# xyfJASON/ctrlora

Measured on NVIDIA H100. Metric: ddim_steps_per_sec, higher is better.
Workload: dtype fp16 (fp32 accumulate)

## Files before the change

ctrlora_b200/csrc/attention_sm90.cu:

```cuda
#include "common.cuh"
#include "ctrlora_b200.h"
#include "wgmma.cuh"
#include <math.h>
#include <string.h>

namespace ctrl {

int make_tmap_f16(CUtensorMap* map, const void* base, int rank, const uint64_t* dims, const uint64_t* strides_bytes,
                  const uint32_t* box);
int persistent_sms();

struct AttnParams {
    int Nq, Nk, heads, d;
    int n_kv_tiles, q_tiles, units;
    float scale_log2e;
    __half* out;
    long long ldo;
    float* lse;
};

constexpr int ATT_BKV = 64;

template <int DP>
struct AttnSmem {
    static constexpr int NWG = DP <= 48 ? 3 : 2;
    static constexpr int BQ = 64 * NWG;
    static constexpr int THREADS = 128 * (NWG + 1), CONSUMERS = 128 * NWG;
    static constexpr int PRODUCER_REGS = NWG == 3 ? 24 : 40, CONSUMER_REGS = NWG == 3 ? 160 : 232;
    static constexpr int NKC = (DP + 63) / 64;
    static constexpr int STAGES = DP <= 48 ? 6 : DP <= 80 ? 4 : 3;
    static constexpr int Q_CHUNK = BQ * 128;
    static constexpr int Q_BYTES = NKC * Q_CHUNK;
    static constexpr int K_CHUNK = ATT_BKV * 128;
    static constexpr int K_BYTES = NKC * K_CHUNK;
    static constexpr int V_BYTES = DP * 128;
    static constexpr int STAGE = K_BYTES + V_BYTES;
    static constexpr int DATA = Q_BYTES + STAGES * STAGE;
    static constexpr int TOTAL = DATA + (2 + 2 * STAGES) * 8 + 1024;
};

template <int DP>
__device__ __forceinline__ void issue_qk(float* s, uint32_t sQ, uint32_t sK) {
    using L = AttnSmem<DP>;
#pragma unroll
    for (int kk = 0; kk < DP / 16; ++kk)
        WgmmaSS<64, 0, 0>::mma(s, wgmma_desc_kmajor(sQ + (kk >> 2) * L::Q_CHUNK + (kk & 3) * 32),
                               wgmma_desc_kmajor(sK + (kk >> 2) * L::K_CHUNK + (kk & 3) * 32), kk ? 1u : 0u);
    wgmma_commit();
}

template <int DP>
__device__ __forceinline__ void issue_pv(float* o, const uint32_t* pa, uint32_t sV) {
#pragma unroll
    for (int kk = 0; kk < 4; ++kk) WgmmaRS<DP, 0>::mma(o, pa + 4 * kk, wgmma_desc_kmajor(sV + 32 * kk), 1u);
    wgmma_commit();
}

template <bool MASK>
__device__ __forceinline__ void softmax_tile(float* s, float (&m)[2], float (&l)[2], float (&a)[2], float c, int key0,
                                             int nk) {
    float mx[2] = {m[0], m[1]};
#pragma unroll
    for (int i = 0; i < 8; ++i)
#pragma unroll
        for (int e = 0; e < 2; ++e) {
            const bool ok = !MASK || key0 + 8 * i + e < nk;
            s[4 * i + e] = ok ? s[4 * i + e] * c : -INFINITY;
            s[4 * i + 2 + e] = ok ? s[4 * i + 2 + e] * c : -INFINITY;
            mx[0] = fmaxf(mx[0], s[4 * i + e]);
            mx[1] = fmaxf(mx[1], s[4 * i + 2 + e]);
        }
    float ls[2] = {0.f, 0.f};
#pragma unroll
    for (int h = 0; h < 2; ++h) {
        mx[h] = fmaxf(mx[h], __shfl_xor_sync(0xffffffffu, mx[h], 1));
        mx[h] = fmaxf(mx[h], __shfl_xor_sync(0xffffffffu, mx[h], 2));
        a[h] = fast_exp2(m[h] - mx[h]);
        m[h] = mx[h];
    }
#pragma unroll
    for (int i = 0; i < 8; ++i)
#pragma unroll
        for (int e = 0; e < 2; ++e) {
            s[4 * i + e] = fast_exp2(s[4 * i + e] - m[0]);
            s[4 * i + 2 + e] = fast_exp2(s[4 * i + 2 + e] - m[1]);
            ls[0] += s[4 * i + e];
            ls[1] += s[4 * i + 2 + e];
        }
    l[0] = l[0] * a[0] + ls[0];
    l[1] = l[1] * a[1] + ls[1];
}

__device__ __forceinline__ void pack_a_frags(const float* x, uint32_t* a) {
#pragma unroll
    for (int i = 0; i < 8; ++i) {
        a[4 * (i >> 1) + 2 * (i & 1)] = pack_half2(x[4 * i], x[4 * i + 1]);
        a[4 * (i >> 1) + 2 * (i & 1) + 1] = pack_half2(x[4 * i + 2], x[4 * i + 3]);
    }
}

template <int DP>
__global__ void __launch_bounds__(AttnSmem<DP>::THREADS, 1)
attention_kernel(const __grid_constant__ CUtensorMap tmQ, const __grid_constant__ CUtensorMap tmK,
                 const __grid_constant__ CUtensorMap tmV, const __grid_constant__ AttnParams p) {
    using L = AttnSmem<DP>;
    extern __shared__ uint8_t smem_raw[];
    uint8_t* smem = reinterpret_cast<uint8_t*>((reinterpret_cast<uintptr_t>(smem_raw) + 1023) & ~uintptr_t(1023));
    uint64_t* q_full = reinterpret_cast<uint64_t*>(smem + L::DATA);
    uint64_t* q_empty = q_full + 1;
    uint64_t* full = q_full + 2;
    uint64_t* empty = full + L::STAGES;
    pdl_launch_dependents();
    const int warp = uniform_warp_idx();
    const int n_kv = p.n_kv_tiles;
    if (threadIdx.x == 0) {
        tma_prefetch_desc(&tmQ);
        tma_prefetch_desc(&tmK);
        tma_prefetch_desc(&tmV);
        mbar_init(q_full, 1);
        mbar_init(q_empty, L::CONSUMERS);
        for (int i = 0; i < L::STAGES; ++i) {
            mbar_init(&full[i], 1);
            mbar_init(&empty[i], L::CONSUMERS);
        }
        fence_barrier_init();
    }
    __syncthreads();
    pdl_wait();

    if (warp < 4) {
        setmaxnreg_dec<L::PRODUCER_REGS>();
        if (warp == 0 && elect_one()) {
            int s = 0;
            uint32_t phase = 0, qphase = 0;
            for (int u = blockIdx.x; u < p.units; u += gridDim.x) {
                const int qt = u % p.q_tiles, hi = u / p.q_tiles, head = hi % p.heads, img = hi / p.heads;
                mbar_wait_nocall(q_empty, qphase ^ 1);
                qphase ^= 1;
                mbar_expect_tx(q_full, L::Q_BYTES);
#pragma unroll
                for (int c = 0; c < L::NKC; ++c)
                    tma_load_4d(smem + c * L::Q_CHUNK, &tmQ, q_full, c * 64, head, qt * L::BQ, img);
                for (int t = 0; t < n_kv; ++t) {
                    mbar_wait_nocall(&empty[s], phase ^ 1);
                    uint8_t* dst = smem + L::Q_BYTES + s * L::STAGE;
                    mbar_expect_tx(&full[s], L::STAGE);
#pragma unroll
                    for (int c = 0; c < L::NKC; ++c)
                        tma_load_4d(dst + c * L::K_CHUNK, &tmK, &full[s], c * 64, head, t * ATT_BKV, img);
                    tma_load_4d(dst + L::K_BYTES, &tmV, &full[s], t * ATT_BKV, 0, head, img);
                    if (++s == L::STAGES) { s = 0; phase ^= 1; }
                }
            }
        }
        return;
    }

    setmaxnreg_inc<L::CONSUMER_REGS>();
    const int ct = threadIdx.x - 128, wg = ct >> 7, lane = threadIdx.x & 31;
    const uint32_t sQ = smem_u32(smem) + wg * 64 * 128, sKV = smem_u32(smem) + L::Q_BYTES;
    const float c = p.scale_log2e;
    const bool ragged = (p.Nk % ATT_BKV) != 0;
    const int kq = 2 * (lane & 3);
    const int bar_own = 1 + wg, bar_next = 1 + (wg + 1) % L::NWG;
    if (wg == L::NWG - 1) named_bar_arrive(1, 256);
    int s = 0;
    uint32_t phase = 0, qphase = 0;
    for (int u = blockIdx.x; u < p.units; u += gridDim.x) {
        const int qt = u % p.q_tiles, hi = u / p.q_tiles, head = hi % p.heads, img = hi / p.heads;
        float o[DP / 2];
#pragma unroll
        for (int i = 0; i < DP / 2; ++i) o[i] = 0.f;
        float m[2] = {-INFINITY, -INFINITY}, l[2] = {0.f, 0.f}, a[2];
        float sc[32];
        uint32_t pa[16];
        mbar_wait_nocall(q_full, qphase);
        qphase ^= 1;

        mbar_wait_nocall(&full[s], phase);
        named_bar_sync(bar_own, 256);
        wgmma_fence();
        issue_qk<DP>(sc, sQ, sKV + s * L::STAGE);
        named_bar_arrive(bar_next, 256);
        wgmma_wait<0>();
        wgmma_fence_regs<32>(sc);
        if (n_kv == 1) mbar_arrive(q_empty);
        if (ragged && n_kv == 1) softmax_tile<true>(sc, m, l, a, c, kq, p.Nk);
        else softmax_tile<false>(sc, m, l, a, c, kq, p.Nk);
        pack_a_frags(sc, pa);
        int prev = s;
        if (++s == L::STAGES) { s = 0; phase ^= 1; }

        for (int t = 1; t < n_kv; ++t) {
            mbar_wait_nocall(&full[s], phase);
            named_bar_sync(bar_own, 256);
            wgmma_fence();
            issue_qk<DP>(sc, sQ, sKV + s * L::STAGE);
            issue_pv<DP>(o, pa, sKV + prev * L::STAGE + L::K_BYTES);
            named_bar_arrive(bar_next, 256);
            wgmma_wait<1>();
            wgmma_fence_regs<32>(sc);
            if (t == n_kv - 1) mbar_arrive(q_empty);
            if (ragged && t == n_kv - 1) softmax_tile<true>(sc, m, l, a, c, t * ATT_BKV + kq, p.Nk);
            else softmax_tile<false>(sc, m, l, a, c, t * ATT_BKV + kq, p.Nk);
            wgmma_wait<0>();
            wgmma_fence_regs<DP / 2>(o);
            wgmma_fence_regs<16>(pa);
            mbar_arrive(&empty[prev]);
            if (__any_sync(0xffffffffu, a[0] != 1.f || a[1] != 1.f)) {
#pragma unroll
                for (int i = 0; i < DP / 8; ++i) {
                    o[4 * i] *= a[0]; o[4 * i + 1] *= a[0];
                    o[4 * i + 2] *= a[1]; o[4 * i + 3] *= a[1];
                }
            }
            pack_a_frags(sc, pa);
            prev = s;
            if (++s == L::STAGES) { s = 0; phase ^= 1; }
        }
        wgmma_fence();
        issue_pv<DP>(o, pa, sKV + prev * L::STAGE + L::K_BYTES);
        wgmma_wait<0>();
        wgmma_fence_regs<DP / 2>(o);
        mbar_arrive(&empty[prev]);

#pragma unroll
        for (int h = 0; h < 2; ++h) {
            l[h] += __shfl_xor_sync(0xffffffffu, l[h], 1);
            l[h] += __shfl_xor_sync(0xffffffffu, l[h], 2);
        }
        const float inv0 = 1.0f / l[0], inv1 = 1.0f / l[1];
        const int r0 = qt * L::BQ + wg * 64 + ((ct >> 5) & 3) * 16 + (lane >> 2), r1 = r0 + 8;
        __half* o0 = p.out + (static_cast<long long>(img) * p.Nq + r0) * p.ldo + head * p.d;
        __half* o1 = p.out + (static_cast<long long>(img) * p.Nq + r1) * p.ldo + head * p.d;
#pragma unroll
        for (int i = 0; i < DP / 8; ++i) {
            const int col = 8 * i + kq;
            if (col >= p.d) continue;
            if (r0 < p.Nq) *reinterpret_cast<__half2*>(o0 + col) = __floats2half2_rn(o[4 * i] * inv0, o[4 * i + 1] * inv0);
            if (r1 < p.Nq) *reinterpret_cast<__half2*>(o1 + col) = __floats2half2_rn(o[4 * i + 2] * inv1, o[4 * i + 3] * inv1);
        }
        if (p.lse && (lane & 3) == 0) {
            float* lrow = p.lse + (static_cast<long long>(img) * p.heads + head) * p.Nq;
            if (r0 < p.Nq) lrow[r0] = m[0] + log2f(l[0]);
            if (r1 < p.Nq) lrow[r1] = m[1] + log2f(l[1]);
        }
    }
    if (wg == 0) named_bar_sync(1, 256);
}

template <int DP>
static int launch_attn(const CUtensorMap& tq, const CUtensorMap& tk, const CUtensorMap& tv, const AttnParams& p, int grid,
                       cudaStream_t stream) {
    using L = AttnSmem<DP>;
    static bool attr = false;
    if (!attr) {
        if (cudaFuncSetAttribute(attention_kernel<DP>, cudaFuncAttributeMaxDynamicSharedMemorySize, L::TOTAL) != cudaSuccess)
            return CTRLORA_ERR_CUDA;
        attr = true;
    }
    if (launch_pdl(attention_kernel<DP>, dim3(grid), dim3(L::THREADS), (size_t)L::TOTAL, stream, tq, tk, tv, p) !=
        cudaSuccess)
        return CTRLORA_ERR_CUDA;
    return cudaGetLastError() == cudaSuccess ? CTRLORA_OK : CTRLORA_ERR_CUDA;
}

}

using namespace ctrl;

extern "C" int ctrlora_attention_f16(const void* q, long long ldq, const void* k, long long ldk, const void* vt,
                                     int nk_pad, void* out, long long ldo, float* lse, int batch, int heads, int nq,
                                     int nk, int head_dim, void* stream_) {
    cudaStream_t stream = reinterpret_cast<cudaStream_t>(stream_);
    if (!q || !k || !vt || !out) return CTRLORA_ERR_ARG;
    const int d = head_dim;
    if (d % 8 != 0 || d > 160 || nk_pad % 8 != 0 || nk_pad < nk || ldq % 8 != 0 || ldk % 8 != 0 || ldo % 8 != 0 || nk < 1)
        return CTRLORA_ERR_ARG;
    const int dp = d <= 48 ? 48 : d <= 80 ? 80 : 160;
    const int bq = dp == 48 ? AttnSmem<48>::BQ : dp == 80 ? AttnSmem<80>::BQ : AttnSmem<160>::BQ;
    AttnParams p;
    memset(&p, 0, sizeof(p));
    p.Nq = nq; p.Nk = nk; p.heads = heads; p.d = d;
    p.n_kv_tiles = (nk + ATT_BKV - 1) / ATT_BKV;
    p.q_tiles = (nq + bq - 1) / bq;
    p.units = p.q_tiles * heads * batch;
    p.scale_log2e = (1.0f / sqrtf(static_cast<float>(d))) * 1.4426950408889634f;
    p.out = reinterpret_cast<__half*>(out); p.ldo = ldo; p.lse = lse;
    if (p.units == 0) return CTRLORA_OK;
    const int sms = persistent_sms();
    if (sms <= 0) return CTRLORA_ERR_CUDA;
    CUtensorMap tq, tk, tv;
    {
        uint64_t dims[4] = {(uint64_t)d, (uint64_t)heads, (uint64_t)nq, (uint64_t)batch};
        uint64_t str[3] = {(uint64_t)d * 2, (uint64_t)ldq * 2, (uint64_t)ldq * 2 * nq};
        uint32_t box[4] = {64, 1, (uint32_t)bq, 1};
        int rc = make_tmap_f16(&tq, q, 4, dims, str, box);
        if (rc) return rc;
    }
    {
        uint64_t dims[4] = {(uint64_t)d, (uint64_t)heads, (uint64_t)nk, (uint64_t)batch};
        uint64_t str[3] = {(uint64_t)d * 2, (uint64_t)ldk * 2, (uint64_t)ldk * 2 * nk};
        uint32_t box[4] = {64, 1, ATT_BKV, 1};
        int rc = make_tmap_f16(&tk, k, 4, dims, str, box);
        if (rc) return rc;
    }
    {
        uint64_t dims[4] = {(uint64_t)nk, (uint64_t)d, (uint64_t)heads, (uint64_t)batch};
        uint64_t str[3] = {(uint64_t)nk_pad * 2, (uint64_t)nk_pad * 2 * d, (uint64_t)nk_pad * 2 * d * heads};
        uint32_t box[4] = {ATT_BKV, (uint32_t)dp, 1, 1};
        int rc = make_tmap_f16(&tv, vt, 4, dims, str, box);
        if (rc) return rc;
    }
    const int grid = p.units < sms ? p.units : sms;
    if (dp == 48) return launch_attn<48>(tq, tk, tv, p, grid, stream);
    if (dp == 80) return launch_attn<80>(tq, tk, tv, p, grid, stream);
    return launch_attn<160>(tq, tk, tv, p, grid, stream);
}
```

ctrlora_b200/ops.py:

```python
import ctypes as C

import torch

from . import _lib
from ._lib import GemmArgs, check


LAUNCHES = 0
_GEMM_PROFILE = None
_GEMM_SHAPES = None
_GEMM_RECORD = None


def _count(n=1):
    global LAUNCHES
    LAUNCHES += n


def _ungraphed(fn, sampler):
    old = getattr(sampler, "use_cuda_graph", False)
    if sampler is not None:
        sampler.use_cuda_graph = False
    try:
        fn()
# ... 157 lines not shown
        assert residual.dtype in (torch.float16, torch.float32) and residual.stride(-1) == 1
        args.residual, args.ldr = _ptr(residual), residual.stride(-2)
        args.residual_f32 = int(residual.dtype == torch.float32)
    args.out_scale, args.head_dim, args.tok_pad, args.bf16 = float(out_scale), head_dim, tok_pad, 0
    ws, cnt = _splitk_buffers(a.device)
    args.split_k, args.splitk_ws, args.splitk_ws_bytes = split_k, ws.data_ptr(), SPLITK_WS_BYTES
    args.splitk_counters, args.splitk_counters_len = cnt.data_ptr(), SPLITK_COUNTERS
    if dup_out is not None:
        args.dup_out, args.dup_ld = dup_out.data_ptr(), dup_out.stride(0)
    args.force_single_cta = int(single_cta)
    args.relu = int(bool(relu))
    if hi is not None:
        if hi.get("rowbias") is not None:
            assert rowbias is not None and hi["rowbias"].stride(0) == rowbias.stride(0) and \
                hi["rowbias"].stride(-1) == 1, "the two halves' row terms need one row stride"
        args.group_b, args.w_hi, args.w2_hi = b // 2, _ptr(hi["w"]), _ptr(hi.get("w2"))
        args.bias_hi, args.rowbias_hi = _ptr(hi.get("bias")), _ptr(hi.get("rowbias"))
    lib = _lib.load()
    shape = {"B": b, "H": h, "W": wd, "C": c, "N": n_rows, "ksize": ksize, "geglu": int(geglu),
             "c2": int(args.a2_c) if a2 is not None else 0, "segs": seg_width, "res": int(residual is not None)}
    keep = (a, w, a2, w2, bias, rowbias, residual, out, seg_outs, dup_out, ws, cnt, hi)
    if _launch_gemm(lib.ctrlora_gemm_f16_simt if simt else lib.ctrlora_gemm_f16, args, simt, shape, keep):
        return ret
    half = a.shape[0] // 2
    rows = half if a.dim() == 2 else half * a.shape[1] * a.shape[2]
    imgs = rows // (rows_per_img or rows)

    def cut(t, lo, by_image=False):
        if t is None:
            return None
        n = imgs if by_image else (half if t.dim() == 4 else rows)
        return t[:n] if lo else t[n:]

    for lo in (True, False):
        segs = None if seg_outs is None else [cut(o, lo, by_image=bool(t)) for o, t in zip(seg_outs, transposed)]
        _gemm(cut(a, lo), w if lo else hi["w"], ksize=ksize, bias=bias if lo else hi.get("bias"),
              rowbias=rowbias if lo else hi.get("rowbias"), rows_per_img=rows_per_img, rowbias_ld=rowbias_ld,
              residual=cut(residual, lo), out_scale=out_scale, a2=cut(a2, lo), w2=w2 if lo else hi.get("w2"),
              geglu=geglu, out=cut(out, lo), out_f32=out_f32, seg_outs=segs, seg_width=seg_width, transposed=transposed,
              head_dim=head_dim, tok_pad=tok_pad, block_n=block_n, split_k=split_k, relu=relu)
    return ret


def _launch_gemm(fn, args, simt, shape, keep):
    flops = 2.0 * shape["B"] * shape["H"] * shape["W"] * shape["N"] * (shape["ksize"] ** 2 * shape["C"] + shape["c2"])
    timed = _GEMM_PROFILE is not None and not simt
    if timed:
        e0, e1 = torch.cuda.Event(enable_timing=True), torch.cuda.Event(enable_timing=True)
        e0.record()
    rc = fn(C.addressof(args), _sp())
    if rc == _lib.STATUS_UNSUPPORTED and args.group_b:
        return False
    check(rc, "ctrlora_gemm_f16")
    _count()
    if _GEMM_RECORD is not None and not simt:
        _GEMM_RECORD.append((args, flops, keep))
    if timed:
        e1.record()
        _GEMM_PROFILE.append((flops, e0, e1))
        if _GEMM_SHAPES is not None:
            _GEMM_SHAPES.append(shape)
    return True


def _dp(t):
    return t.data_ptr() if t is not None else None


def _sp():
    return torch.cuda.current_stream().cuda_stream


_GN_PARTIAL = {}
GN_PARTIAL_FLOATS = 1 << 19
GN_PARTIAL_COUNTERS = 256


def _gn_partial_buffers(device):
    key = device.index if device.index is not None else torch.cuda.current_device()
    if key not in _GN_PARTIAL:
        if torch.cuda.is_current_stream_capturing():
            raise _lib.CtrloraError("the GroupNorm partial-statistics scratch is allocated on the first call on a device; "
                                    "make one un-captured GroupNorm call before capturing a graph")
        _GN_PARTIAL[key] = (torch.empty(GN_PARTIAL_FLOATS, device=device, dtype=torch.float32),
                            torch.zeros(GN_PARTIAL_COUNTERS, device=device, dtype=torch.int32))
    return _GN_PARTIAL[key]


def _gn_args(x1, gamma, beta, eps, silu, add1, add1_scale, x2, add2, add2_scale, groups):
    b, h, w, c1, ld1 = _as_bhwc(x1)
    c2, ld2 = 0, 0
    if x2 is not None:
        b2, h2, w2, c2, ld2 = _as_bhwc(x2)
        assert (b2, h2, w2) == (b, h, w)
    a = _lib.GroupNormArgs()
    a.x1, a.add1, a.add1_scale, a.c1, a.ld1 = _dp(x1), _dp(add1), float(add1_scale), c1, ld1
    a.x2, a.add2, a.add2_scale, a.c2, a.ld2 = _dp(x2), _dp(add2), float(add2_scale), c2, ld2
    a.batch, a.hw, a.groups = b, h * w, groups
    a.gamma, a.beta, a.eps, a.silu = _dp(gamma), _dp(beta), float(eps), int(silu)
    pws, pcnt = _gn_partial_buffers(x1.device)
    a.partial_ws, a.partial_ws_floats = _dp(pws), GN_PARTIAL_FLOATS
    a.partial_counters, a.partial_counters_len = _dp(pcnt), GN_PARTIAL_COUNTERS
    return a, (b, h, w, c1, c2)


def groupnorm(x1, gamma, beta, eps, silu, *, add1=None, add1_scale=1.0, x2=None, add2=None, add2_scale=1.0,
              groups=32, want_raw=False, want_stats=False, out=None, gamma_hi=None, beta_hi=None):
    _require_cuda(x1, x2, add1, add2)
    a, (b, h, w, c1, c2) = _gn_args(x1, gamma, beta, eps, silu, add1, add1_scale, x2, add2, add2_scale, groups)
    for ad, ref in ((add1, x1), (add2, x2)):
        if ad is not None:
            assert ad.shape == ref.shape and ad.stride() == ref.stride() and ad.dtype == torch.float16
    ctot = c1 + c2
    y = torch.empty((b, h, w, ctot), device=x1.device, dtype=torch.float16) if out is None else out
    assert y.shape == (b, h, w, ctot) and y.is_contiguous() and y.dtype == torch.float16
    raw = torch.empty_like(y) if want_raw else None
    stats_ws = torch.empty(b * groups * 2, device=x1.device, dtype=torch.float32)
    a.stats_ws = _dp(stats_ws)
    assert gamma.dtype == torch.float32 and beta.dtype == torch.float32 and gamma.numel() == ctot
    if gamma_hi is not None:
        assert b % 2 == 0 and gamma_hi.numel() == ctot and beta_hi.numel() == ctot
        a.gamma_hi, a.beta_hi, a.group_b = _dp(gamma_hi), _dp(beta_hi), b // 2
    a.y, a.raw_out = _dp(y), _dp(raw)
    _count(2)
    check(_lib.load().ctrlora_groupnorm_f16(C.addressof(a), _sp()), "ctrlora_groupnorm_f16")
    if want_stats:
        return (y, raw, stats_ws) if want_raw else (y, stats_ws)
    return (y, raw) if want_raw else y


def zeros(shape, device, dtype=torch.float16):
    t = torch.empty(shape, device=device, dtype=dtype)
    check(_lib.load().ctrlora_memset_zero(_dp(t), t.numel() * t.element_size(), _sp()), "memset_zero")
    return t


def layernorm(x, gamma, beta, eps=1e-5, gamma_hi=None, beta_hi=None):
    _require_cuda(x)
    cols = x.shape[-1]
    x2 = x.reshape(-1, cols)
    y = torch.empty((x2.shape[0], cols), device=x.device, dtype=torch.float16)
    _count(1)
    if gamma_hi is not None:
        assert x2.shape[0] % 2 == 0
        check(_lib.load().ctrlora_layernorm_grouped_f16(_dp(x2), x2.stride(0), _dp(y), cols, x2.shape[0], cols, _dp(gamma),
                                                        _dp(beta), _dp(gamma_hi), _dp(beta_hi), x2.shape[0] // 2,
                                                        float(eps), _sp()), "ctrlora_layernorm_grouped_f16")
        return y.view(x.shape)
    check(_lib.load().ctrlora_layernorm_f16(_dp(x2), x2.stride(0), _dp(y), cols, x2.shape[0], cols, _dp(gamma), _dp(beta),
                                            float(eps), _sp()), "ctrlora_layernorm_f16")
    return y.view(x.shape)


def attention(q, k, vt, batch, heads, nq, nk, head_dim, out=None, lse=None):
    _require_cuda(q, k, vt)
    if out is None:
        out = torch.empty((batch * nq, heads * head_dim), device=q.device, dtype=torch.float16)
    _count(1)
    check(_lib.load().ctrlora_attention_f16(_dp(q), q.stride(0), _dp(k), k.stride(0), _dp(vt), vt.shape[-1], _dp(out),
                                            out.stride(0), _dp(lse), batch, heads, nq, nk, head_dim, _sp()),
          "ctrlora_attention_f16")
    return out


def nchw_to_nhwc_f16(x, c_pad=None, out=None):
    _require_cuda(x)
    assert x.dtype == torch.float32 and x.is_contiguous()
    b, c, h, w = x.shape
    c_pad = c_pad or c
    y = torch.empty((b, h, w, c_pad), device=x.device, dtype=torch.float16) if out is None else out
    assert y.shape == (b, h, w, c_pad) and y.is_contiguous() and y.dtype == torch.float16
    _count(1)
    check(_lib.load().ctrlora_nchw_f32_to_nhwc_f16(_dp(x), _dp(y), b, c, h * w, c_pad, _sp()), "nchw_to_nhwc")
    return y


def nhwc_to_nchw_f32(x, channels=None):
    _require_cuda(x)
    b, h, w, c, ld = _as_bhwc(x)
    channels = channels or c
    y = torch.empty((b, channels, h, w), device=x.device, dtype=torch.float32)
    _count(1)
    check(_lib.load().ctrlora_nhwc_to_nchw_f32(_dp(x), int(x.dtype == torch.float32), ld, _dp(y), b, channels, h * w,
                                               _sp()), "nhwc_to_nchw")
    return y


def timestep_embedding(t, freqs):
    _require_cuda(t, freqs)
    assert t.dtype in (torch.int64, torch.float32) and freqs.dtype == torch.float32
    out = torch.empty((t.shape[0], 2 * freqs.shape[0]), device=t.device, dtype=torch.float32)
    fn = _lib.load().ctrlora_timestep_embedding if t.dtype == torch.int64 else _lib.load().ctrlora_timestep_embedding_f32
    _count(1)
    check(fn(_dp(t), _dp(freqs), _dp(out), t.shape[0], freqs.shape[0], _sp()), "timestep_embedding")
    return out


def small_linear(x, w, bias, silu_in=False, silu_out=False, out=None):
    _require_cuda(x, w)
    assert x.dtype == torch.float32 and w.dtype == torch.float16 and w.is_contiguous() and x.stride(1) == 1
    rows, k = x.shape
    n = w.shape[0]
    if out is None:
        out = torch.empty((rows, n), device=x.device, dtype=torch.float32)
    _count(1)
    check(_lib.load().ctrlora_small_linear(_dp(x), x.stride(0), _dp(w), _dp(bias), _dp(out), out.stride(0), rows, n, k,
                                           int(silu_in), int(silu_out), _sp()), "small_linear")
    return out


def upsample2x(x):
    _require_cuda(x)
    assert x.is_contiguous() and x.dtype == torch.float16
    b, h, w, c = x.shape
    y = torch.empty((b, 2 * h, 2 * w, c), device=x.device, dtype=torch.float16)
    _count(1)
    check(_lib.load().ctrlora_upsample2x_f16(_dp(x), _dp(y), b, h, w, c, _sp()), "upsample2x")
    return y


def im2col_s2(x, pad_lo=1):
    _require_cuda(x)
    assert x.is_contiguous() and x.dtype == torch.float16
    b, h, w, c = x.shape
    y = torch.empty((b, h // 2, w // 2, 9 * c), device=x.device, dtype=torch.float16)
    _count(1)
    check(_lib.load().ctrlora_im2col_s2_pad_f16(_dp(x), _dp(y), b, h, w, c, int(pad_lo), _sp()), "im2col_s2")
    return y


def softmax_rows(logits, scale=1.0):
    _require_cuda(logits)
    assert logits.dtype == torch.float32 and logits.dim() == 2 and logits.stride(1) == 1
    out = torch.empty(logits.shape, device=logits.device, dtype=torch.float16)
    _count(1)
    check(_lib.load().ctrlora_softmax_rows_f32_to_f16(_dp(logits), logits.stride(0), _dp(out), out.stride(0), logits.shape[0],
                                                      logits.shape[1], float(scale), _sp()), "softmax_rows")
    return out


def gaussian_sample(moments, noise=None, scale=1.0):
    _require_cuda(moments, noise)
    moments = moments.float().contiguous()
    b, z2, h, w = moments.shape
    out = torch.empty((b, z2 // 2, h, w), device=moments.device, dtype=torch.float32)
    if noise is not None:
        noise = noise.float().contiguous()
        assert noise.shape == out.shape
    _count(1)
    check(_lib.load().ctrlora_gaussian_sample(_dp(moments), _dp(noise), _dp(out), b, z2 // 2, h * w, float(scale), _sp()),
          "gaussian_sample")
    return out


def cast_transpose(src, batch, rows, cols, out=None):
    _require_cuda(src)
    assert src.dtype == torch.float32 and src.is_contiguous() and src.numel() == batch * rows * cols
    if out is None:
        out = torch.empty((batch, cols, rows), device=src.device, dtype=torch.float16)
    _count(1)
    check(_lib.load().ctrlora_cast_transpose_f32_to_f16(_dp(src), _dp(out), batch, rows, cols, _sp()), "cast_transpose")
    return out


def ddim_update(x, e_cond, e_uncond, cfg_scale, a_t, a_prev, sigma_t, sqrt_one_minus_at, noise=None, temperature=1.0,
                stats=None):
    _require_cuda(x, e_cond, e_uncond, noise)
    for t in (x, e_cond, e_uncond, noise):
        assert t is None or (t.dtype == torch.float32 and t.is_contiguous() and t.shape == x.shape)
    x_prev, pred_x0 = torch.empty_like(x), torch.empty_like(x)
    b = x.shape[0]
    _count(1)
    check(_lib.load().ctrlora_ddim_update(_dp(x), _dp(e_cond), _dp(e_uncond), _dp(noise), _dp(x_prev), _dp(pred_x0),
                                          _dp(stats), b, x[0].numel(), float(cfg_scale), float(a_t), float(a_prev),
                                          float(sigma_t), float(sqrt_one_minus_at), float(temperature), _sp()),
          "ddim_update")
    return x_prev, pred_x0


def im2col_3x3(x):
    _require_cuda(x)
    assert x.is_contiguous() and x.dtype == torch.float16
    b, h, w, c = x.shape
    y = torch.empty((b, h, w, 9 * c), device=x.device, dtype=torch.float16)
    _count()
    check(_lib.load().ctrlora_im2col_3x3_f16(_dp(x), _dp(y), b, h, w, c, _sp()), "im2col_3x3")
    return y


def outer_accum(dy, x, out, alpha=1.0, beta=1.0, silu_x=False):
    _require_cuda(dy, x, out)
    assert dy.dtype == x.dtype == out.dtype == torch.float32 and dy.stride(1) == 1 and x.stride(1) == 1 and out.stride(1) == 1
    rows, n = dy.shape
    k = x.shape[1]
    assert x.shape[0] == rows and out.shape == (n, k)
    _count()
    check(_lib.load().ctrlora_outer_accum_f32(_dp(dy), dy.stride(0), _dp(x), x.stride(0), _dp(out), out.stride(0), rows, n, k,
                                              float(alpha), float(beta), int(silu_x), _sp()), "outer_accum")
    return out


def copy2d(src, dst, rows, cols, lds, ldd, accumulate=False):
    _require_cuda(src, dst)
    assert src.dtype == dst.dtype == torch.float32
    _count()
    check(_lib.load().ctrlora_copy2d_f32(_dp(src), lds, _dp(dst), ldd, rows, cols, int(accumulate), _sp()), "copy2d")
    return dst


def silu_bwd(d, x):
# ... 704 lines not shown
```

ctrlora_b200/train.py:

```python
import numbers
import os

import torch
import torch.nn as nn

from . import checkpoint, ops, prepare
from .runtime import nchw_view, pixel_major, to_f16_rows

f32 = prepare.bias_f32


class GradSink:

    def __init__(self, control_model, named=None):
        if named is None:
            from cldm.cldm_ctrlora_finetune import trainable_parameters
            if not getattr(control_model, "ft_with_lora", True):
                raise NotImplementedError("FinetuneTrainer covers ft_with_lora=True; use PretrainTrainer (dense weight "
                                          "gradients of every ControlNet parameter) for full-parameter training")
            named = trainable_parameters(control_model)
        self.names = [n for n, _ in named]
        self.params = [p for _, p in named]
        total = sum(p.numel() for p in self.params)
        dev = self.params[0].device
# ... 364 lines not shown
    from ldm.modules.diffusionmodules.openaimodel import Downsample, ResBlock, Upsample, _Conv
    tape = []
    for layer in seq:
        if isinstance(layer, ResBlock):
            x, s = res_fwd(layer, x, emb.slices[id(layer)])
            tape.append(("res", layer, s))
        elif isinstance(layer, SpatialTransformer):
            x, s = st_fwd(layer, x, ctx)
            tape.append(("st", layer, s))
        elif isinstance(layer, Downsample):
            x, s = down_fwd(layer, x)
            tape.append(("down", layer, s))
        elif isinstance(layer, Upsample):
            x, s = up_fwd(layer, x)
            tape.append(("up", layer, s))
        elif isinstance(layer, _Conv):
            cin = layer.in_channels
            c_pad = (cin + 7) // 8 * 8
            xin = pixel_major(x, c_pad if c_pad != cin else None)
            x = layer(nchw_view(xin))
            tape.append(("stop", layer, {"xin": xin}))
        else:
            raise NotImplementedError(type(layer))
    return x, tape


def seq_bwd(tape, d, G, emb_grads=None, first_res_kw=None):
    for i in range(len(tape) - 1, -1, -1):
        kind, mod, s = tape[i]
        if kind == "res":
            kw = first_res_kw if (i == 0 and first_res_kw) else {}
            rg = emb_grads.get(id(mod)) if emb_grads is not None else None
            d = res_bwd(mod, s, d, rowbias_grad=rg, G=G, **kw)
        elif kind == "st":
            d = st_bwd(mod, s, d, G)
        elif kind == "down":
            d = down_bwd(mod, s, d, G)
        elif kind == "up":
            d = up_bwd(mod, s, d)
        elif kind == "stop":
            if G is not None:
                dense_conv_grads(mod, s["xin"], pixel_major(d), G)
            return None
    return d


def _small_lora_grads(lin, x, dy, G, silu_x=False):
    gw, gb = G.grad(lin.weight), G.grad(getattr(lin, "bias", None))
    if gw is not None:
        ops.outer_accum(dy, x, gw, silu_x=silu_x)
    if gb is not None:
        ops.colsum(dy, gb)
    lora = getattr(lin, "lora_layer", None)
    if lora is None:
        return
    gu, gd = G.grad(lora.up.weight), G.grad(lora.down.weight)
    if gu is None:
        return
    sc = 1.0 if lora.network_alpha is None else lora.network_alpha / lora.rank
    r, k = lora.down.weight.shape
    n = lora.up.weight.shape[0]
    c = _cache(lora)
    d16 = c.get("d16s", [lora.down.weight], lambda: prepare.linear_weight(lora.down.weight).view(r, k))
    u16t = c.get("u16ts", [lora.up.weight], lambda: ops.cast_transpose(f32(lora.up.weight), 1, n, r).view(r, n))
    t1 = ops.small_linear(x, d16, None, silu_in=silu_x)
    ops.outer_accum(dy, t1, gu, alpha=sc)
    t2 = ops.small_linear(dy, u16t, None)
    ops.outer_accum(t2, x, gd, alpha=sc, silu_x=silu_x)


def emb_mlp_backward(net, t_emb, emb, d_all, slices, G):
    from ldm.modules.diffusionmodules.openaimodel import ResBlock
    blocks = [m for m in net.modules() if isinstance(m, ResBlock)]
    l0, l2 = net.time_embed[0], net.time_embed[2]
    for rb in blocks:
        _small_lora_grads(rb.emb_layers[1], emb, slices[id(rb)], G, silu_x=True)
    lins = [b.emb_layers[1] for b in blocks]
    params = [p for lin in lins for p in prepare.linear_params(lin)]
    wcat_t = _cache(net).get("emb_cat_T", params, lambda: prepare.weight_T(
        torch.cat([b.emb_weight() for b in blocks], 0).contiguous().view(-1, 1, l2.out_features)).view(l2.out_features, -1))
    d_se = ops.small_linear(d_all, wcat_t, None)
    d_emb = ops.silu_bwd(d_se, emb)
    w0 = _cache(l0).get("w2d", prepare.linear_params(l0), lambda: prepare.effective_linear_weight(l0).view(l0.out_features, -1))
    hid_pre = ops.small_linear(t_emb, w0, f32(l0.bias))
    _small_lora_grads(l2, hid_pre, d_emb, G, silu_x=True)
    w2t = _cache(l2).get("w2dT", prepare.linear_params(l2), lambda: prepare.weight_T(
        prepare.effective_linear_weight(l2)).view(l2.in_features, l2.out_features))
    d_hid = ops.small_linear(d_emb, w2t, None)
    d_hid_pre = ops.silu_bwd(d_hid, hid_pre)
    _small_lora_grads(l0, t_emb, d_hid_pre, G)


def controlnet_fwd(cn, hint, t, ctx):
    emb = cn.embed(t)
    ctx16 = to_f16_rows(ctx).view(ctx.shape[0], ctx.shape[1], -1)
    tapes, hs, outs = [], [], []
    h = hint
    for module, zc in zip(cn.input_blocks, cn.zero_convs):
        h, tape = seq_fwd(module, h, emb, ctx16)
        tapes.append(tape)
        hs.append(h)
        outs.append(cn._zero_conv(zc, h))
    h, tape = seq_fwd(cn.middle_block, h, emb, ctx16)
    tapes.append(tape)
    hs.append(h)
    outs.append(cn._zero_conv(cn.middle_block_out, h))
    return outs, {"tapes": tapes, "hs": hs, "emb": emb, "t": t}


def zero_conv_bwd(seq, h, d_out, G, upstream):
    conv = prepare.effective(seq[0])
    hp, dp = pixel_major(h), pixel_major(d_out)
    b, hh, ww, c = hp.shape
    h2d, d2d = hp.reshape(b * hh * ww, c), dp.reshape(b * hh * ww, c)
    gw, gb = G.grad(conv.weight), G.grad(conv.bias)
    if gw is not None:
        ops.wgrad_tn(d2d, h2d, out=gw.view(c, c), beta=1.0)
        ops.colsum(d2d, gb)
    wt = _cache(conv).get("wT", [conv.weight], lambda: prepare.weight_T(prepare.conv_weight(conv.weight)))
    up = None if upstream is None else pixel_major(upstream).reshape(b * hh * ww, c)
    return nchw_view(ops.gemm(dp, wt, residual=up))


STAGE_AFTER_BLOCK = {9: "ib9", 6: "ib6", 3: "ib3"}


def controlnet_bwd(cn, saved, d_outs, G, on_stage=None):
    from ldm.modules.diffusionmodules.openaimodel import ResBlock
    emb = saved["emb"]
    bsz = emb.raw.shape[0]
    blocks = [m for m in cn.modules() if isinstance(m, ResBlock)]
    d_all = torch.zeros((bsz, sum(b.out_channels for b in blocks)), device=emb.raw.device, dtype=torch.float32)
    emb_grads, off = {}, 0
    for b in blocks:
        emb_grads[id(b)] = d_all[:, off:off + b.out_channels]
        off += b.out_channels
    tapes, hs = saved["tapes"], saved["hs"]
    d_h = zero_conv_bwd(cn.middle_block_out, hs[-1], d_outs[-1], G, None)
    d_h = seq_bwd(tapes[-1], d_h, G, emb_grads)
    if on_stage is not None:
        on_stage("middle")
    for i in range(len(cn.input_blocks) - 1, -1, -1):
        d_h = zero_conv_bwd(cn.zero_convs[i], hs[i], d_outs[i], G, d_h)
        d_h = seq_bwd(tapes[i], d_h, G, emb_grads)
        if on_stage is not None and i in STAGE_AFTER_BLOCK:
            on_stage(STAGE_AFTER_BLOCK[i])
    from ldm.modules.diffusionmodules.util import timestep_embedding
    t_emb = timestep_embedding(saved["t"], cn.model_channels)
    emb_mlp_backward(cn, t_emb, emb.raw, d_all, emb_grads, G)


def unet_fwd(unet, x, t, ctx, control, scales, only_mid_control=False):
    from .runtime import CatSpec
    with torch.no_grad():
        emb = unet.embed(t)
        ctx16 = to_f16_rows(ctx).view(ctx.shape[0], ctx.shape[1], -1)
        hs = []
        h = x
        for module in unet.input_blocks:
            h = module(h, emb, ctx16)
            hs.append(h)
        h = unet.middle_block(h, emb, ctx16)
    ctrl = list(zip(control, scales))
    add_mid, s_mid = ctrl.pop()
    tapes = []
    for i, module in enumerate(unet.output_blocks):
        skip = hs.pop()
        add, sc = (None, 1.0) if only_mid_control else ctrl.pop()
        spec = CatSpec(h, add1=add_mid if i == 0 else None, s1=s_mid, x2=skip, add2=add, s2=sc)
        h, tape = seq_fwd(module, spec, emb, ctx16)
        tapes.append(tape)
    gn, conv = unet.out[0], unet.out[2]
    hp = pixel_major(h)
    a, stats = ops.groupnorm(hp, f32(gn.weight), f32(gn.bias), gn.eps, True, want_stats=True)
    n_pad = (unet.out_channels + 15) // 16 * 16
    bias = unet._prep.get("out_bias", [conv.bias], lambda: torch.cat(
        [conv.bias.detach().float(), torch.zeros(n_pad - unet.out_channels, device=conv.bias.device)]).contiguous())
    y = ops.gemm(a, conv.kernel_weight(pad_out=n_pad), ksize=3, bias=bias, out_f32=True)
    eps = ops.nhwc_to_nchw_f32(y, unet.out_channels)
    return eps, {"tapes": tapes, "hp": hp, "stats": stats, "n_pad": n_pad, "only_mid": only_mid_control}


def unet_bwd(unet, saved, d_eps16):
    gn, conv = unet.out[0], unet.out[2]
    wd = _cache(conv).get("wd_out", [conv.weight],
                          lambda: prepare.conv_dgrad_weight(conv.kernel_weight(pad_out=saved["n_pad"])))
    d_a = ops.gemm(d_eps16, wd, ksize=3)
    d_h = nchw_view(ops.groupnorm_bwd(d_a, saved["stats"], saved["hp"], f32(gn.weight), f32(gn.bias), gn.eps, True))
    d_ctrl = []
    tapes = saved["tapes"]
    for i in range(len(tapes) - 1, -1, -1):
        want2 = not saved["only_mid"]
        if i == 0:
            src = tapes[0][0][2]["src"]
            res = seq_bwd(tapes[0], d_h, None, None, first_res_kw=dict(want_dx2=want2, dx1_scale=src["add1_scale"]))
        else:
            res = seq_bwd(tapes[i], d_h, None, None, first_res_kw=dict(want_dx2=want2))
        if want2:
            d_h, d2 = res
            d_ctrl.append(d2)
        else:
            d_h = res
    d_ctrl = d_ctrl[::-1] if d_ctrl else []
    ordered = [None] * 13
    for j, g in enumerate(d_ctrl):
        ordered[11 - j] = g
    ordered[12] = d_h
    return ordered


class FinetuneTrainer:

    tasks = ()

    def __init__(self, model, lr=1e-5, betas=(0.9, 0.999), eps=1e-8, weight_decay=0.01, process_group=None,
                 loss_scale=None, dynamic_loss_scale=True, accumulate_grad_batches=1, *, named=None):
        self._init_window(accumulate_grad_batches)
        self.model = model
        self.cn = model.control_model
        self.unet = model.model.diffusion_model
        self.G = GradSink(self.cn, named=named)
        self.lr, self.betas, self.eps, self.wd = lr, betas, eps, weight_decay
        self.pg = process_group
        self.world, self.rank = 1, 0
        if torch.distributed.is_available() and torch.distributed.is_initialized():
            self.world = torch.distributed.get_world_size(process_group)
            self.rank = torch.distributed.get_rank(process_group)
        if self.world > 1:
            torch.distributed.broadcast(self.G.flat_p, src=0, group=process_group)
            prepare.bump_train_version()
        self.step_count = 0
        self.seg_steps = {}
        self.loss_scale = loss_scale
        self.dynamic_loss_scale = dynamic_loss_scale
        dev = self.G.flat_p.device
        self.overflow_flag = torch.zeros(1, device=dev, dtype=torch.int32)
        self.skipped_steps = 0
        self._init_step_state(dev)
        self._graphs = None
        self._static = None
        self._on_stage = None
        self._comm = None

    LOSS_SCALE_DIV = 8.0
    CHECK_OVERFLOW_EVERY = 16

    def _init_window(self, k):
        if isinstance(k, bool) or not isinstance(k, numbers.Integral) or k < 1:
            raise ValueError(f"accumulate_grad_batches must be an integer >= 1, got {k!r}")
        self.accumulate_grad_batches = int(k)
        self.micro_step = 0
        self._window_tasks = []

    def _init_step_state(self, dev):
        self._step_dev = {}
        self._bc_dev = {}
        self._skipped_dev = torch.zeros(1, device=dev, dtype=torch.int32)
        self._skipped_seen = 0
        self._launched = 0

    def _seg_state(self, key):
        if key not in self._step_dev:
            dev = self.G.flat_p.device
            self._step_dev[key] = torch.zeros(1, device=dev, dtype=torch.int32)
            self._bc_dev[key] = torch.ones(2, device=dev, dtype=torch.float32)
        return self._step_dev[key], self._bc_dev[key]

    def _poll_overflow(self, force=False):
        self._launched += 1
        if not (force or (self.dynamic_loss_scale and self._launched % self.CHECK_OVERFLOW_EVERY == 0)):
            return False
        skipped = int(self._skipped_dev.item())
        if skipped == self._skipped_seen:
            return False
        self.skipped_steps += skipped - self._skipped_seen
        self._skipped_seen = skipped
        self.loss_scale = self._scale_used * 0.5
        return True

    def _scale_for(self, numel):
        return float(self.loss_scale) if self.loss_scale is not None else numel / (2.0 * self.LOSS_SCALE_DIV)

    def loss_and_grads(self, x0, hint_latent, context, t, noise, task=None, accumulate=False):
        m = self.model
        if task is not None and self.tasks:
            self.cn.switch_lora(task)
            self.task = task
        if not accumulate:
            self.G.zero()
            self.overflow_flag.zero_()
            self._scale_used = self._scale_for(x0.numel())
        x_noisy = m.q_sample(x_start=x0, t=t, noise=noise)
        control, cn_saved = controlnet_fwd(self.cn, hint_latent, t, context)
        eps, un_saved = unet_fwd(self.unet, x_noisy, t, context, control, m.control_scales, m.only_mid_control)
        loss, d_eps = ops.mse_loss_grad(eps, noise, c_pad=un_saved["n_pad"], grad_scale=self._scale_used)
        d_ctrl = unet_bwd(self.unet, un_saved, d_eps)
        if m.only_mid_control:
            d_ctrl = [d if d is not None else torch.zeros_like(c) for d, c in zip(d_ctrl, control)]
        controlnet_bwd(self.cn, cn_saved, d_ctrl, self.G, on_stage=self._on_stage)
        self.last_eps = eps
        return loss

    def unscaled_grads(self):
        inv = 1.0 / self._scale_used
        return {n: g * inv for n, g in self.G.named_grads().items()}

    STAGES = ("middle",) + tuple(STAGE_AFTER_BLOCK.values())
# ... 424 lines not shown
```

Before: 37.30.

## Add lean inference attention path with folded scaling, double-buffered Q, and ones-column row sums

Adds a LEAN template variant of the attention kernel, used when no log-sum-exp output is requested (inference). It folds the softmax scale into one fmaf before exp2, skips the rescale exp when the running max does not move, and double-buffers Q tiles for head dims up to 80. For d<48 it writes a column of ones into the padded V tile so the PV tensor-core MMA produces the row sums, removing the per-tile scalar sum. Training forward passes force the old path by allocating lse through a context manager. The cost is more template instantiations, extra shared memory and barriers, and a subtle dependence on the padded V columns staying intact.

Result: faster. 37.98 (median of 6 runs) (+1.8%).

```diff
diff --git a/ctrlora_b200/csrc/attention_sm90.cu b/ctrlora_b200/csrc/attention_sm90.cu
--- a/ctrlora_b200/csrc/attention_sm90.cu
+++ b/ctrlora_b200/csrc/attention_sm90.cu
@@ -21,13 +21,14 @@
 
 constexpr int ATT_BKV = 64;
 
-template <int DP>
+template <int DP, int NQB = 1>
 struct AttnSmem {
     static constexpr int NWG = DP <= 48 ? 3 : 2;
     static constexpr int BQ = 64 * NWG;
     static constexpr int THREADS = 128 * (NWG + 1), CONSUMERS = 128 * NWG;
     static constexpr int PRODUCER_REGS = NWG == 3 ? 24 : 40, CONSUMER_REGS = NWG == 3 ? 160 : 232;
     static constexpr int NKC = (DP + 63) / 64;
+    static constexpr int QB = NQB;
     static constexpr int STAGES = DP <= 48 ? 6 : DP <= 80 ? 4 : 3;
     static constexpr int Q_CHUNK = BQ * 128;
     static constexpr int Q_BYTES = NKC * Q_CHUNK;
@@ -35,9 +36,11 @@
     static constexpr int K_BYTES = NKC * K_CHUNK;
     static constexpr int V_BYTES = DP * 128;
     static constexpr int STAGE = K_BYTES + V_BYTES;
-    static constexpr int DATA = Q_BYTES + STAGES * STAGE;
-    static constexpr int TOTAL = DATA + (2 + 2 * STAGES) * 8 + 1024;
+    static constexpr int DATA = QB * Q_BYTES + STAGES * STAGE;
+    static constexpr int TOTAL = DATA + (2 * QB + 2 * STAGES) * 8 + 1024;
 };
+
+__host__ __device__ constexpr int attn_qbufs(int DP, bool LEAN) { return LEAN && DP <= 80 ? 2 : 1; }
 
 template <int DP>
 __device__ __forceinline__ void issue_qk(float* s, uint32_t sQ, uint32_t sK) {
@@ -91,6 +94,59 @@
     l[1] = l[1] * a[1] + ls[1];
 }
 
+template <bool MASK, bool SUMS>
+__device__ __forceinline__ bool softmax_tile_lean(float* s, float (&m)[2], float (&l)[2], float (&a)[2], float c,
+                                                  int key0, int nk) {
+    if (MASK) {
+#pragma unroll
+        for (int i = 0; i < 8; ++i)
+#pragma unroll
+            for (int e = 0; e < 2; ++e)
+                if (key0 + 8 * i + e >= nk) s[4 * i + e] = s[4 * i + 2 + e] = -INFINITY;
+    }
+    float mx[2];
+#pragma unroll
+    for (int h = 0; h < 2; ++h) {
+        float t[8];
+#pragma unroll
+        for (int i = 0; i < 8; ++i) t[i] = fmaxf(s[4 * i + 2 * h], s[4 * i + 2 * h + 1]);
+#pragma unroll
+        for (int w = 4; w >= 1; w >>= 1)
+#pragma unroll
+            for (int i = 0; i < w; ++i) t[i] = fmaxf(t[i], t[i + w]);
+        mx[h] = fmaxf(m[h], t[0]);
+        mx[h] = fmaxf(mx[h], __shfl_xor_sync(0xffffffffu, mx[h], 1));
+        mx[h] = fmaxf(mx[h], __shfl_xor_sync(0xffffffffu, mx[h], 2));
+    }
+    const bool moved = __any_sync(0xffffffffu, mx[0] != m[0] || mx[1] != m[1]);
+#pragma unroll
+    for (int h = 0; h < 2; ++h) {
+        a[h] = moved ? fast_exp2((m[h] - mx[h]) * c) : 1.f;
+        m[h] = mx[h];
+    }
+    const float mc0 = -m[0] * c, mc1 = -m[1] * c;
+#pragma unroll
+    for (int i = 0; i < 8; ++i)
+#pragma unroll
+        for (int e = 0; e < 2; ++e) {
+            s[4 * i + e] = fast_exp2(fmaf(s[4 * i + e], c, mc0));
+            s[4 * i + 2 + e] = fast_exp2(fmaf(s[4 * i + 2 + e], c, mc1));
+        }
+    if (SUMS) {
+        float ls[2] = {0.f, 0.f};
+#pragma unroll
+        for (int i = 0; i < 8; ++i)
+#pragma unroll
+            for (int e = 0; e < 2; ++e) {
+                ls[0] += s[4 * i + e];
+                ls[1] += s[4 * i + 2 + e];
+            }
+        l[0] = l[0] * a[0] + ls[0];
+        l[1] = l[1] * a[1] + ls[1];
+    }
+    return moved;
+}
+
 __device__ __forceinline__ void pack_a_frags(const float* x, uint32_t* a) {
 #pragma unroll
     for (int i = 0; i < 8; ++i) {
@@ -99,16 +155,17 @@
     }
 }
 
-template <int DP>
-__global__ void __launch_bounds__(AttnSmem<DP>::THREADS, 1)
+template <int DP, bool LEAN>
+__global__ void __launch_bounds__(AttnSmem<DP, attn_qbufs(DP, LEAN)>::THREADS, 1)
 attention_kernel(const __grid_constant__ CUtensorMap tmQ, const __grid_constant__ CUtensorMap tmK,
                  const __grid_constant__ CUtensorMap tmV, const __grid_constant__ AttnParams p) {
-    using L = AttnSmem<DP>;
+    using L = AttnSmem<DP, attn_qbufs(DP, LEAN)>;
+    constexpr bool ONES = LEAN && DP == 48;
     extern __shared__ uint8_t smem_raw[];
     uint8_t* smem = reinterpret_cast<uint8_t*>((reinterpret_cast<uintptr_t>(smem_raw) + 1023) & ~uintptr_t(1023));
     uint64_t* q_full = reinterpret_cast<uint64_t*>(smem + L::DATA);
-    uint64_t* q_empty = q_full + 1;
-    uint64_t* full = q_full + 2;
+    uint64_t* q_empty = q_full + L::QB;
+    uint64_t* full = q_full + 2 * L::QB;
     uint64_t* empty = full + L::STAGES;
     pdl_launch_dependents();
     const int warp = uniform_warp_idx();
@@ -117,13 +174,25 @@
         tma_prefetch_desc(&tmQ);
         tma_prefetch_desc(&tmK);
         tma_prefetch_desc(&tmV);
-        mbar_init(q_full, 1);
-        mbar_init(q_empty, L::CONSUMERS);
+        for (int i = 0; i < L::QB; ++i) {
+            mbar_init(&q_full[i], 1);
+            mbar_init(&q_empty[i], L::CONSUMERS);
+        }
         for (int i = 0; i < L::STAGES; ++i) {
             mbar_init(&full[i], 1);
             mbar_init(&empty[i], L::CONSUMERS);
         }
         fence_barrier_init();
+    }
+    if (ONES) {
+        const int per_stage = (DP - p.d) * 8;
+        const uint32_t base = smem_u32(smem) + L::QB * L::Q_BYTES + L::K_BYTES + p.d * 128;
+        for (int j = threadIdx.x; j < L::STAGES * per_stage; j += L::THREADS) {
+            const int st = j / per_stage, r = j - st * per_stage;
+            const uint32_t v = r < 8 ? 0x3C003C00u : 0u;
+            sts128(base + st * L::STAGE + r * 16, v, v, v, v);
+        }
+        fence_proxy_async_smem();
     }
     __syncthreads();
     pdl_wait();
@@ -133,18 +202,21 @@
         if (warp == 0 && elect_one()) {
             int s = 0;
             uint32_t phase = 0, qphase = 0;
+            int qb = 0;
             for (int u = blockIdx.x; u < p.units; u += gridDim.x) {
                 const int qt = u % p.q_tiles, hi = u / p.q_tiles, head = hi % p.heads, img = hi / p.heads;
-                mbar_wait_nocall(q_empty, qphase ^ 1);
-                qphase ^= 1;
-                mbar_expect_tx(q_full, L::Q_BYTES);
+                const int qbuf = L::QB == 1 ? 0 : qb;
+                mbar_wait_nocall(&q_empty[qbuf], qphase ^ 1);
+                mbar_expect_tx(&q_full[qbuf], L::Q_BYTES);
 #pragma unroll
                 for (int c = 0; c < L::NKC; ++c)
-                    tma_load_4d(smem + c * L::Q_CHUNK, &tmQ, q_full, c * 64, head, qt * L::BQ, img);
+                    tma_load_4d(smem + qbuf * L::Q_BYTES + c * L::Q_CHUNK, &tmQ, &q_full[qbuf], c * 64, head, qt * L::BQ,
+                                img);
+                if (L::QB == 1 || ++qb == L::QB) { qb = 0; qphase ^= 1; }
                 for (int t = 0; t < n_kv; ++t) {
                     mbar_wait_nocall(&empty[s], phase ^ 1);
-                    uint8_t* dst = smem + L::Q_BYTES + s * L::STAGE;
-                    mbar_expect_tx(&full[s], L::STAGE);
+                    uint8_t* dst = smem + L::QB * L::Q_BYTES + s * L::STAGE;
+                    mbar_expect_tx(&full[s], ONES ? L::K_BYTES + p.d * 128 : L::STAGE);
 #pragma unroll
                     for (int c = 0; c < L::NKC; ++c)
                         tma_load_4d(dst + c * L::K_CHUNK, &tmK, &full[s], c * 64, head, t * ATT_BKV, img);
@@ -158,7 +230,7 @@
 
     setmaxnreg_inc<L::CONSUMER_REGS>();
     const int ct = threadIdx.x - 128, wg = ct >> 7, lane = threadIdx.x & 31;
-    const uint32_t sQ = smem_u32(smem) + wg * 64 * 128, sKV = smem_u32(smem) + L::Q_BYTES;
+    const uint32_t sQ0 = smem_u32(smem) + wg * 64 * 128, sKV = smem_u32(smem) + L::QB * L::Q_BYTES;
     const float c = p.scale_log2e;
     const bool ragged = (p.Nk % ATT_BKV) != 0;
     const int kq = 2 * (lane & 3);
@@ -166,6 +238,7 @@
     if (wg == L::NWG - 1) named_bar_arrive(1, 256);
     int s = 0;
     uint32_t phase = 0, qphase = 0;
+    int qb = 0;
     for (int u = blockIdx.x; u < p.units; u += gridDim.x) {
         const int qt = u % p.q_tiles, hi = u / p.q_tiles, head = hi % p.heads, img = hi / p.heads;
         float o[DP / 2];
@@ -174,8 +247,10 @@
         float m[2] = {-INFINITY, -INFINITY}, l[2] = {0.f, 0.f}, a[2];
         float sc[32];
         uint32_t pa[16];
-        mbar_wait_nocall(q_full, qphase);
-        qphase ^= 1;
+        const int qbuf = L::QB == 1 ? 0 : qb;
+        const uint32_t sQ = sQ0 + qbuf * L::Q_BYTES;
+        mbar_wait_nocall(&q_full[qbuf], qphase);
+        if (L::QB == 1 || ++qb == L::QB) { qb = 0; qphase ^= 1; }
 
         mbar_wait_nocall(&full[s], phase);
         named_bar_sync(bar_own, 256);
@@ -184,9 +259,14 @@
         named_bar_arrive(bar_next, 256);
         wgmma_wait<0>();
         wgmma_fence_regs<32>(sc);
-        if (n_kv == 1) mbar_arrive(q_empty);
-        if (ragged && n_kv == 1) softmax_tile<true>(sc, m, l, a, c, kq, p.Nk);
-        else softmax_tile<false>(sc, m, l, a, c, kq, p.Nk);
+        if (n_kv == 1) mbar_arrive(&q_empty[qbuf]);
+        if constexpr (LEAN) {
+            if (ragged && n_kv == 1) softmax_tile_lean<true, !ONES>(sc, m, l, a, c, kq, p.Nk);
+            else softmax_tile_lean<false, !ONES>(sc, m, l, a, c, kq, p.Nk);
+        } else {
+            if (ragged && n_kv == 1) softmax_tile<true>(sc, m, l, a, c, kq, p.Nk);
+            else softmax_tile<false>(sc, m, l, a, c, kq, p.Nk);
+        }
         pack_a_frags(sc, pa);
         int prev = s;
         if (++s == L::STAGES) { s = 0; phase ^= 1; }
@@ -200,14 +280,20 @@
             named_bar_arrive(bar_next, 256);
             wgmma_wait<1>();
             wgmma_fence_regs<32>(sc);
-            if (t == n_kv - 1) mbar_arrive(q_empty);
-            if (ragged && t == n_kv - 1) softmax_tile<true>(sc, m, l, a, c, t * ATT_BKV + kq, p.Nk);
-            else softmax_tile<false>(sc, m, l, a, c, t * ATT_BKV + kq, p.Nk);
+            if (t == n_kv - 1) mbar_arrive(&q_empty[qbuf]);
+            bool moved = false;
+            if constexpr (LEAN) {
+                moved = ragged && t == n_kv - 1 ? softmax_tile_lean<true, !ONES>(sc, m, l, a, c, t * ATT_BKV + kq, p.Nk)
+                                                : softmax_tile_lean<false, !ONES>(sc, m, l, a, c, t * ATT_BKV + kq, p.Nk);
+            } else {
+                if (ragged && t == n_kv - 1) softmax_tile<true>(sc, m, l, a, c, t * ATT_BKV + kq, p.Nk);
+                else softmax_tile<false>(sc, m, l, a, c, t * ATT_BKV + kq, p.Nk);
+            }
             wgmma_wait<0>();
             wgmma_fence_regs<DP / 2>(o);
             wgmma_fence_regs<16>(pa);
             mbar_arrive(&empty[prev]);
-            if (__any_sync(0xffffffffu, a[0] != 1.f || a[1] != 1.f)) {
+            if (LEAN ? moved : __any_sync(0xffffffffu, a[0] != 1.f || a[1] != 1.f)) {
 #pragma unroll
                 for (int i = 0; i < DP / 8; ++i) {
                     o[4 * i] *= a[0]; o[4 * i + 1] *= a[0];
@@ -224,10 +310,18 @@
         wgmma_fence_regs<DP / 2>(o);
         mbar_arrive(&empty[prev]);
 
-#pragma unroll
-        for (int h = 0; h < 2; ++h) {
-            l[h] += __shfl_xor_sync(0xffffffffu, l[h], 1);
-            l[h] += __shfl_xor_sync(0xffffffffu, l[h], 2);
+        if constexpr (ONES) {
+#pragma unroll
+            for (int i = 0; i < DP / 8; ++i)
+                if (8 * i == p.d) { l[0] = o[4 * i]; l[1] = o[4 * i + 2]; }
+#pragma unroll
+            for (int h = 0; h < 2; ++h) l[h] = __shfl_sync(0xffffffffu, l[h], lane & ~3);
+        } else {
+#pragma unroll
+            for (int h = 0; h < 2; ++h) {
+                l[h] += __shfl_xor_sync(0xffffffffu, l[h], 1);
+                l[h] += __shfl_xor_sync(0xffffffffu, l[h], 2);
+            }
         }
         const float inv0 = 1.0f / l[0], inv1 = 1.0f / l[1];
         const int r0 = qt * L::BQ + wg * 64 + ((ct >> 5) & 3) * 16 + (lane >> 2), r1 = r0 + 8;
@@ -240,7 +334,7 @@
             if (r0 < p.Nq) *reinterpret_cast<__half2*>(o0 + col) = __floats2half2_rn(o[4 * i] * inv0, o[4 * i + 1] * inv0);
             if (r1 < p.Nq) *reinterpret_cast<__half2*>(o1 + col) = __floats2half2_rn(o[4 * i + 2] * inv1, o[4 * i + 3] * inv1);
         }
-        if (p.lse && (lane & 3) == 0) {
+        if (!LEAN && p.lse && (lane & 3) == 0) {
             float* lrow = p.lse + (static_cast<long long>(img) * p.heads + head) * p.Nq;
             if (r0 < p.Nq) lrow[r0] = m[0] + log2f(l[0]);
             if (r1 < p.Nq) lrow[r1] = m[1] + log2f(l[1]);
@@ -249,17 +343,17 @@
     if (wg == 0) named_bar_sync(1, 256);
 }
 
-template <int DP>
+template <int DP, bool LEAN>
 static int launch_attn(const CUtensorMap& tq, const CUtensorMap& tk, const CUtensorMap& tv, const AttnParams& p, int grid,
                        cudaStream_t stream) {
-    using L = AttnSmem<DP>;
+    using L = AttnSmem<DP, attn_qbufs(DP, LEAN)>;
     static bool attr = false;
     if (!attr) {
-        if (cudaFuncSetAttribute(attention_kernel<DP>, cudaFuncAttributeMaxDynamicSharedMemorySize, L::TOTAL) != cudaSuccess)
+        if (cudaFuncSetAttribute(attention_kernel<DP, LEAN>, cudaFuncAttributeMaxDynamicSharedMemorySize, L::TOTAL) != cudaSuccess)
             return CTRLORA_ERR_CUDA;
         attr = true;
     }
-    if (launch_pdl(attention_kernel<DP>, dim3(grid), dim3(L::THREADS), (size_t)L::TOTAL, stream, tq, tk, tv, p) !=
+    if (launch_pdl(attention_kernel<DP, LEAN>, dim3(grid), dim3(L::THREADS), (size_t)L::TOTAL, stream, tq, tk, tv, p) !=
         cudaSuccess)
         return CTRLORA_ERR_CUDA;
     return cudaGetLastError() == cudaSuccess ? CTRLORA_OK : CTRLORA_ERR_CUDA;
@@ -278,6 +372,7 @@
     if (d % 8 != 0 || d > 160 || nk_pad % 8 != 0 || nk_pad < nk || ldq % 8 != 0 || ldk % 8 != 0 || ldo % 8 != 0 || nk < 1)
         return CTRLORA_ERR_ARG;
     const int dp = d <= 48 ? 48 : d <= 80 ? 80 : 160;
+    const bool lean = lse == nullptr && (dp != 48 || d < 48);
     const int bq = dp == 48 ? AttnSmem<48>::BQ : dp == 80 ? AttnSmem<80>::BQ : AttnSmem<160>::BQ;
     AttnParams p;
     memset(&p, 0, sizeof(p));
@@ -308,12 +403,12 @@
     {
         uint64_t dims[4] = {(uint64_t)nk, (uint64_t)d, (uint64_t)heads, (uint64_t)batch};
         uint64_t str[3] = {(uint64_t)nk_pad * 2, (uint64_t)nk_pad * 2 * d, (uint64_t)nk_pad * 2 * d * heads};
-        uint32_t box[4] = {ATT_BKV, (uint32_t)dp, 1, 1};
+        uint32_t box[4] = {ATT_BKV, (uint32_t)(lean && dp == 48 ? d : dp), 1, 1};
         int rc = make_tmap_f16(&tv, vt, 4, dims, str, box);
         if (rc) return rc;
     }
     const int grid = p.units < sms ? p.units : sms;
-    if (dp == 48) return launch_attn<48>(tq, tk, tv, p, grid, stream);
-    if (dp == 80) return launch_attn<80>(tq, tk, tv, p, grid, stream);
-    return launch_attn<160>(tq, tk, tv, p, grid, stream);
-}
+    if (dp == 48) return lean ? launch_attn<48, true>(tq, tk, tv, p, grid, stream) : launch_attn<48, false>(tq, tk, tv, p, grid, stream);
+    if (dp == 80) return lean ? launch_attn<80, true>(tq, tk, tv, p, grid, stream) : launch_attn<80, false>(tq, tk, tv, p, grid, stream);
+    return lean ? launch_attn<160, true>(tq, tk, tv, p, grid, stream) : launch_attn<160, false>(tq, tk, tv, p, grid, stream);
+}
diff --git a/ctrlora_b200/ops.py b/ctrlora_b200/ops.py
--- a/ctrlora_b200/ops.py
+++ b/ctrlora_b200/ops.py
@@ -333,10 +333,26 @@
     return y.view(x.shape)
 
 
+_TRAINING_SOFTMAX = False
+
+
+class training_softmax:
+
+    def __enter__(self):
+        global _TRAINING_SOFTMAX
+        self._prev, _TRAINING_SOFTMAX = _TRAINING_SOFTMAX, True
+
+    def __exit__(self, *exc):
+        global _TRAINING_SOFTMAX
+        _TRAINING_SOFTMAX = self._prev
+
+
 def attention(q, k, vt, batch, heads, nq, nk, head_dim, out=None, lse=None):
     _require_cuda(q, k, vt)
     if out is None:
         out = torch.empty((batch * nq, heads * head_dim), device=q.device, dtype=torch.float16)
+    if lse is None and _TRAINING_SOFTMAX:
+        lse = torch.empty((batch, heads, nq), device=q.device, dtype=torch.float32)
     _count(1)
     check(_lib.load().ctrlora_attention_f16(_dp(q), q.stride(0), _dp(k), k.stride(0), _dp(vt), vt.shape[-1], _dp(out),
                                             out.stride(0), _dp(lse), batch, heads, nq, nk, head_dim, _sp()),
diff --git a/ctrlora_b200/train.py b/ctrlora_b200/train.py
--- a/ctrlora_b200/train.py
+++ b/ctrlora_b200/train.py
@@ -540,7 +540,7 @@
 
 def unet_fwd(unet, x, t, ctx, control, scales, only_mid_control=False):
     from .runtime import CatSpec
-    with torch.no_grad():
+    with torch.no_grad(), ops.training_softmax():
         emb = unet.embed(t)
         ctx16 = to_f16_rows(ctx).view(ctx.shape[0], ctx.shape[1], -1)
         hs = []
```
